# awslabs/aws-c-compression

Measured on AMD Instinct MI355X. Metric: GiB/s input consumed, encode+decode, 1 GiB random bytes; % HBM roofline, higher is better.
Workload: dtype u8

## Files before the change

aws-c-compression_amd/csrc/hip/decode_sync_kernels.hip:

```cpp
#include "decode_common.hpp"
#include "launch_common.hpp"

namespace {


template <u32 NS>
__device__ __forceinline__ void dec_sync_chunk(
    const hufd_tables &tb,
    const hufd_dec_item *items,
    const u32 *chunk_item,
    const u8 *d_in,
    u16 *fn_tab,
    u16 *cp_tab,
    u32 *chunk_fn,
    u8 *chunk_regular,
    u32 c) {

    const u32 ns = tb.n_states;
    u32 *timg = reinterpret_cast<u32 *>(dyn_lds);
    u16 *ftab = reinterpret_cast<u16 *>(timg);
    u32 *gtab = timg + kChunkWords;
    u16 *lut = reinterpret_cast<u16 *>(gtab + kGroups * ns);

    const u32 lane = threadIdx.x;
// ... 108 lines not shown
    __syncthreads();
    HUFD_STAMP(0, 4);
#pragma unroll
    for (u32 s = 0; s < NS; ++s) {
        if (s < ns) {
            ftab[s * HUFD_DEC_LANES + lane] = fn[s];
            fn_tab[((u64)c * ns + s) * HUFD_DEC_LANES + lane] = fn[s];
        }
    }
    {
        u16 *cp = cp_tab + (u64)c * kCpRows * HUFD_DEC_LANES + lane;
#pragma unroll
        for (u32 qq = 0; qq + 1 < kQuarters; ++qq) {
            const u32 tail = ref_steps - cp_steps[qq];
            cp[qq * HUFD_DEC_LANES] =
                (u16)(cp_ok[qq] ? 0x8000u | ((cp_pos[qq] - (qq + 1) * kQuarterBits) << 11) | tail : 0u);
        }
        u32 merged = 0;
#pragma unroll
        for (u32 s = 0; s < NS; ++s) {
            merged |= (have_ref && pos[s] != kDead) ? 1u << s : 0u;
        }
        const u32 common = have_ref ? (ref_stop ? kExitStop : ref_exit) : kExitNoRef;
        cp[(kQuarters - 1) * HUFD_DEC_LANES] = (u16)(merged | (common << 12));
    }
    __syncthreads();

    if (lane < kGroups * ns) {
        const u32 g = lane / ns, start = lane % ns;
        gtab[g * ns + start] = wide_pack(chain_fold(kGroupLanes, start, [&](u32 i, u32 stt) {
            return widen(ftab[stt * HUFD_DEC_LANES + g * kGroupLanes + i]);
        }));
    }
    __syncthreads();
    if (lane < ns) {
        chunk_fn[(u64)c * ns + lane] =
            wide_pack(chain_fold(kGroups, lane, [&](u32 g, u32 stt) { return gtab[g * ns + stt]; }));
    }
    HUFD_STAMP(0, 5);
}

template <u32 NS>
__global__ __launch_bounds__(HUFD_DEC_LANES) void dec_sync_kernel(
    hufd_tables tb,
    const hufd_dec_item *items,
    const u32 *chunk_item,
    u32 n_chunks,
    const u8 *d_in,
    u16 *fn_tab,
    u16 *cp_tab,
    u32 *chunk_fn,
    u8 *chunk_regular,
    const u32 *list,
    const u32 *list_count,
    u32 *clear ) {
    if (clear && blockIdx.x == 0 && threadIdx.x == 0) {
        clear[HUFK_DEC_COUNT_EMIT] = 0;
        clear[HUFK_DEC_COUNT_DENSE] = 0;
    }
    const u32 n = list ? *list_count : n_chunks;
    for (u32 i = blockIdx.x; i < n; i += gridDim.x) {
        const u32 c = list ? list[i] : i;
        if (list && chunk_regular[c] == kRegularFew) {
            continue;
        }
        dec_sync_chunk<NS>(tb, items, chunk_item, d_in, fn_tab, cp_tab, chunk_fn, chunk_regular, c);
        __syncthreads();
    }
}

template <u32 LB>
struct lean_shared {
    u32 wlut[1u << LB];
    u32 exit_state[HUFD_DEC_LANES];
    u32 sub0[kFastMaxMeet + 4];
    u32 wave_sum[HUFD_DEC_LANES / 64];
    u32 bad;
    u32 pad[3];
    u16 hops[1u << LB];
};



constexpr u32 kOneRecs = 9;
__device__ __host__ constexpr u32 one_rec_row(u32 j) {
    return j == 0 ? 6u : j == 1 ? 8u : j == 2 ? 10u : j == 3 ? 12u : j == 4 ? 16u : j == 5 ? 20u : j == 6 ? 24u : j == 7 ? 28u : 32u;
}
constexpr u32 kOneMaxMerge = kSubWords;
constexpr u32 kOneMaxMerge0 = kSubWords;
constexpr u32 kOneRecs0 = kOneRecs;
constexpr u32 kOneGarbageRow = 4, kOneGarbageDead = 48;

__device__ __host__ constexpr u32 one_rec_index(u32 row) {
    u32 at = kOneRecs;
    for (u32 j = 0; j < kOneRecs; ++j) {
        at = one_rec_row(j) == row ? j : at;
    }
    return at;
}

struct one_walk {
    u32 thr, mask;
    static constexpr u32 kPos = 0xFFu;
    __device__ __forceinline__ one_walk(u32 lut_bits) {
        thr = 64 + 31;
        mask = ((1u << lut_bits) - 1u) << 2;
    }
    __device__ __forceinline__ u32 state_at(u32 k) const {
        return thr + 32 - k;
    }
    __device__ __forceinline__ u32 offset_of(u32 state) const {
        return thr + 32 - (state & kPos);
    }
    static __device__ __forceinline__ u32 count_of(u32 state) {
        return state >> 19;
    }
    static __device__ __forceinline__ u32 dead_of(u32 state) {
        return (state >> 8) & 0x7FFu;
    }
    static __device__ __forceinline__ u32 entry_of(u32 len) {
        return len ? (1u << 19) - len : (1u << 8) - 1u;
    }
    template <u32 LB>
    static __device__ __forceinline__ u32 shifted(u32 before, u32 word) {
        return funnel(before, word, 31u - LB);
    }
    __device__ __forceinline__ u32 look(u32 state, u32 xh, u32 xl, u32 table) const {
        return lds_word_at((funnel_by_low5(xh, xl, state) & mask) | table);
    }
    template <u32 SURE>
    __device__ __forceinline__ u32 row(u32 state, u32 xh, u32 xl, u32 table) const {
#pragma unroll
        for (u32 i = 0; i < SURE; ++i) {
            state += look(state, xh, xl, table);
        }
        return byte_rows_uncertain(state, xh, xl, table, mask, thr);
    }
};

template <u32 LB>
struct one_shared {
    u32 wlut[1u << LB];
    u32 exit_state[HUFD_DEC_LANES];
    u32 sub0[kSubWords + 4];
    u32 last0;
    u32 tiny[kTailWords];
    u32 wave_sum[HUFD_DEC_LANES / 64];
    u32 bad;
    u32 decided0;
    u32 moved;
    u32 bad_mine;

};

template <u32 LB, u32 SURE, bool TAIL = false>
__global__ __launch_bounds__(HUFD_DEC_LANES, 8) void dec_sync_one_kernel(
    hufd_tables tb,
    const hufd_chunk_rec *chunk_rec,
    const u32 *tail_chunks,
    const u8 *d_in,
    u16 *fn_tab,
    u16 *cp_tab,
    u32 *chunk_fn,
    u16 *lane_count,
    u8 *chunk_regular,
    u32 *tail_entry,
    u32 *slow_list,
    u32 *slow_count,
    u32 *long_list,
    u32 *long_count) {
    constexpr bool FOLLOW = false;
    const u32 c = TAIL ? wave_uniform(tail_chunks[blockIdx.x]) : blockIdx.x;
#include "decode_sync_one_body.inc"
}

template <u32 LB, u32 SURE>
__global__ __launch_bounds__(HUFD_DEC_LANES, 8) void dec_sync_one_mixed_kernel(
    hufd_tables tb,
    const hufd_chunk_rec *chunk_rec,
    const u32 *tail_chunks,
    u32 n_tail,
    const u8 *d_in,
    u16 *fn_tab,
    u16 *cp_tab,
    u32 *chunk_fn,
    u16 *lane_count,
    u8 *chunk_regular,
    u32 *tail_entry,
    u32 *slow_list,
    u32 *slow_count,
    u32 *long_list,
    u32 *long_count) {
    if (blockIdx.x < n_tail) {
        constexpr bool TAIL = true, FOLLOW = true;
        const u32 c = wave_uniform(tail_chunks[blockIdx.x]);
#include "decode_sync_one_body.inc"
    } else {
        constexpr bool TAIL = false, FOLLOW = false;
        const u32 c = blockIdx.x - n_tail;
#include "decode_sync_one_body.inc"
    }
}




template <u32 LB>
struct pack_shared {
    u32 wlut[1u << LB];
    u32 exit_state[HUFD_DEC_LANES];
    u32 sub0[kPackMaxSlots][kFastMaxMeet + 4];
    u32 sum[kPackMaxSlots];
    u32 bad[kPackMaxSlots];
    u32 alive[kPackMaxSlots];
    u32 meet0[kPackMaxSlots];
    u32 tail0[kPackMaxSlots];
    u16 hops[1u << LB];
};

template <u32 LB, u32 SURE>
__global__ __launch_bounds__(HUFD_DEC_LANES, 6) void dec_sync_pack_kernel(
    hufd_tables tb,
    const hufd_chunk_rec *chunk_rec,
    const u32 *tail_chunks,
    u32 n_tail,
    u32 width,
    const u8 *d_in,
    u16 *fn_tab,
    u16 *cp_tab,
    u32 *chunk_fn,
    u16 *lane_count,
    u8 *chunk_regular,
    u32 *tail_entry,
    u32 *long_list,
    u32 *long_count) {
// ... 998 lines not shown
```

aws-c-compression_amd/csrc/hip/decode_sync_one_body.inc:

```

    static_assert(TAIL || !FOLLOW, "only a chunk its stream ends in has an end to follow");
    HUFD_STAMP(0, 0);
    one_shared<LB> &sh = *reinterpret_cast<one_shared<LB> *>(dyn_lds);
    const u32 ns = tb.n_states;
    const u32 lane = threadIdx.x;
    const hufd_chunk_rec rec = chunk_rec[c];
    const u64 valid = rec.valid;
    const u8 *src = d_in + rec.src_off;
    if (!TAIL && valid < (u64)HUFD_DEC_CHUNK_BYTES + 8u) {
        return;
    }
    const u32 n_full = !TAIL ? HUFD_DEC_LANES : (valid >= 8u ? (u32)((valid - 8u) / HUFD_DEC_SUB_BYTES) : 0u);
    const bool active = !TAIL || lane < n_full;
    if (TAIL && n_full == 0 && tb.lut_bits <= HUFD_DEC_MAX_LUT_BITS) {
        if (lane == 0) {
            chunk_regular[c] = 3;
        }
        if (FOLLOW) {
            u16 *lut = reinterpret_cast<u16 *>(sh.wlut);
            for (u32 i = lane; i < (1u << tb.lut_bits); i += HUFD_DEC_LANES) {
                lut[i] = tb.dec_lut[i];
            }
            __syncthreads();
            if (lane == 0) {
                u32 *tiny = sh.tiny;
                load_be32_run(tiny, src, valid, kTailWords);
                const bool only = rec.entry_bit != HUFD_NONE32;
                for (u32 st = only ? rec.entry_bit : 0u; st < (only ? rec.entry_bit + 1u : ns); ++st) {
                    u32 stop_pos = 0, stop_why = 0;
                    const tail_walk tw = tail_follow(tiny, lut, tb.lut_bits, st, (u32)(valid * 8), 2 * HUFD_DEC_SUB_BITS, nullptr, &stop_pos, &stop_why);
                    chunk_fn[(u64)c * ns + st] = wide_pack(true, 0, tw.count[0] + tw.count[1]);
                }
            }
        }
        return;
    }
    const one_walk ow(LB);
    u32 table = lds_offset_of(sh.wlut);
    opaque(table);
    const bool eligible = n_full >= 1 && tb.lut_bits <= LB && tb.max_bits <= HUFD_DEC_MAX_LUT_BITS &&
                          row_walk(LB, tb.max_bits).sure >= SURE && (table & ((4u << LB) - 1u)) == 0;
    if (!eligible) {
        if (lane == 0) {
            chunk_regular[c] = 0;
            long_list[atomicAdd(long_count, 1u)] = c;
        }
        return;
    }
    u16 *cp = cp_tab + (u64)c * kCpRows * HUFD_DEC_LANES + lane;
    constexpr u32 kLutPerLane = (1u << LB) / HUFD_DEC_LANES, kLutBatch = 4;
    const auto table_share = [&](u32 j0) {
        u32 lut_raw[kLutBatch];
#pragma unroll
        for (u32 j = 0; j < kLutBatch; ++j) {
            lut_raw[j] = tb.dec_lut[(lane + (j0 + j) * HUFD_DEC_LANES) >> (LB - tb.lut_bits)];
        }
#pragma unroll
        for (u32 j = 0; j < kLutBatch; ++j) {
            sh.wlut[lane + (j0 + j) * HUFD_DEC_LANES] = one_walk::entry_of(lut_raw[j] & 0xFFu);
        }
    };
    if (TAIL && lane >= kWave && (lane & ~(kWave - 1)) >= n_full) {
#pragma unroll
        for (u32 j0 = 0; j0 < kLutPerLane; j0 += kLutBatch) {
            table_share(j0);
        }
        if (!FOLLOW || (lane != n_full && lane != n_full + 1)) {
#pragma unroll
            for (u32 qq = 0; qq + 1 < kQuarters; ++qq) {
                cp[qq * HUFD_DEC_LANES] = 0;
            }
            lane_count[(u64)c * HUFD_DEC_LANES + lane] = 0;
            cp[(kQuarters - 1) * HUFD_DEC_LANES] = (u16)(kExitStop << 12);
        }
        return;
    }
    u32 w[kFastRows];
    {
        const u32 mine = active ? lane : 0u;
        const unaligned_uint4 *line = reinterpret_cast<const unaligned_uint4 *>(src + (u64)mine * HUFD_DEC_SUB_BYTES);
#pragma unroll
        for (u32 q = 0; q < kSubWords / 4; ++q) {
            const unaligned_uint4 v = line[q];
            w[4 * q + 0] = v.x;
            w[4 * q + 1] = v.y;
            w[4 * q + 2] = v.z;
            w[4 * q + 3] = v.w;
        }
        w[kSubWords] = reinterpret_cast<const unaligned_u32 *>(src + (u64)(mine + 1) * HUFD_DEC_SUB_BYTES)->x;
    }
#pragma unroll
    for (u32 j0 = 0; j0 < kLutPerLane; j0 += kLutBatch) {
        table_share(j0);
    }
    if (lane == 0) {
        sh.bad = 0;
        sh.decided0 = 0;
        sh.moved = 0;
        sh.bad_mine = 0;
#pragma unroll
        for (u32 wv = 0; wv < HUFD_DEC_LANES / kWave; ++wv) {
            sh.wave_sum[wv] = 0;
        }
    }
    {
        u32 behind = __builtin_bswap32(w[kFastRows - 1]);
#pragma unroll
        for (u32 r = kFastRows - 1; r >= 1; --r) {
            const u32 front = __builtin_bswap32(w[r - 1]);
            w[r] = one_walk::shifted<LB>(front, behind);
            behind = front;
        }
        w[0] = one_walk::shifted<LB>(0u, behind);
    }
    if (lane == 0) {
#pragma unroll
        for (u32 r = 0; r <= kOneMaxMerge0; ++r) {
            sh.sub0[r] = w[r];
        }
    }
    __syncthreads();
    HUFD_STAMP(0, 1);
    HUFD_STAMP(0, 2);

    u32 kept_r[kOneRecs + kQuarters - 1];
#pragma unroll
    for (u32 q = 0; q < kOneRecs + kQuarters - 1; ++q) {
        kept_r[q] = 0;
    }
    auto kept_set = [&](u32 q, u32 v) { kept_r[q] = v; };
    auto kept_get = [&](u32 q) -> u32 { return kept_r[q]; };

    u32 state = ow.state_at(0);
    bool hopeless = false;
#pragma unroll
    for (u32 r = 0; r < kSubWords; ++r) {
        if (!hopeless) {
            if (one_rec_index(r) < kOneRecs) {
                kept_set(one_rec_index(r), state);
            }
            if (r != 0 && r % (kSubWords / kQuarters) == 0) {
                kept_set(kOneRecs + r / (kSubWords / kQuarters) - 1, state);
            }
            state = ow.template row<SURE>(state, w[r], w[r + 1], table) + 32u;
            if (r + 1 == kOneGarbageRow) {
                hopeless = __any(active && one_walk::dead_of(state) > kOneGarbageDead);
            }
        }
    }
    const u32 last = state;
    kept_set(kOneRecs - 1, last);
    if (lane == 0) {
        sh.last0 = last;
    }
    u32 ref_exit = ow.offset_of(last);
    bool ok = !hopeless;
    bool ok_mine = !active || ref_exit < ns;
    sh.exit_state[lane] = ref_exit;
    HUFD_STAMP(0, 3);
    __syncthreads();
    HUFD_STAMP(0, 4);

    u32 entry = lane ? sh.exit_state[lane - 1] : 0u;
    u32 count = 0, meet_row = 0;
    u32 head_cp[kQuarters - 1] = {0, 0, 0};
    {
        u32 st = ow.state_at(entry < ns ? entry : 0u);
        bool met = !active || lane == 0;
        u32 h_at = 0, r_at = 0;
        bool done = false;
        constexpr u32 kInRegisters = 24;
#pragma unroll
        for (u32 r = 0; r <= kInRegisters; ++r) {
            if (!done && !hopeless) {
                if (r != 0 && r % (kSubWords / kQuarters) == 0) {
                    head_cp[r / (kSubWords / kQuarters) - 1] = st;
                }
                if (one_rec_index(r) < kOneRecs) {
                    const u32 there = kept_get(one_rec_index(r));
                    if (!met && ((st ^ there) & one_walk::kPos) == 0) {
                        met = true;
                        h_at = st;
                        r_at = there;
                        meet_row = r;
                    }
                    done = __all(met);
                    if (one_rec_index(r) == 0) {
                        if (!done) {
                            hopeless = __popcll(__ballot(!met)) > kWave - kWave / 8;
                        }
                    }
                }
                if (r < kInRegisters) {
                    if (!done && !hopeless) {
                        st = ow.template row<SURE>(st, w[r], w[r + 1], table) + 32u;
                    }
                }
            }
        }
        if (!done && !hopeless) {
            const u8 *mine = src + (u64)(active ? lane : 0u) * HUFD_DEC_SUB_BYTES;
            u32 word = __builtin_bswap32(reinterpret_cast<const unaligned_u32 *>(mine + 4 * kInRegisters)->x);
            u32 hi = one_walk::shifted<LB>(__builtin_bswap32(reinterpret_cast<const unaligned_u32 *>(mine + 4 * (kInRegisters - 1))->x), word);
            for (u32 r = kInRegisters; r < kSubWords && !done; ++r) {
                const u32 next = __builtin_bswap32(reinterpret_cast<const unaligned_u32 *>(mine + 4 * (r + 1))->x);
                const u32 lo = one_walk::shifted<LB>(word, next);
                word = next;
                st = ow.template row<0>(st, hi, lo, table) + 32u;
                hi = lo;
                if (r + 1 == one_rec_row(kOneRecs - 2) || r + 1 == one_rec_row(kOneRecs - 1)) {
                    const u32 there = r + 1 == one_rec_row(kOneRecs - 2) ? kept_get(kOneRecs - 2) : kept_get(kOneRecs - 1);
                    if (!met && ((st ^ there) & one_walk::kPos) == 0) {
                        met = true;
                        h_at = st;
                        r_at = there;
                        meet_row = r + 1;
                    }
                    done = __all(met);
                }
            }
        }
        if (active && lane && !hopeless && !met && entry < ns) {
            met = true;
            h_at = st;
            r_at = last;
            meet_row = kSubWords;
            ref_exit = ow.offset_of(st);
            sh.exit_state[lane] = ref_exit;
            sh.moved = 1;
        }
        if (active && lane) {
            ok_mine = !hopeless && met && entry < ns && ref_exit < ns && one_walk::dead_of(h_at) == 0 &&
                      one_walk::dead_of(last) == one_walk::dead_of(r_at);
            count = one_walk::count_of(h_at) + one_walk::count_of(last) - one_walk::count_of(r_at);
        }
    }

    HUFD_STAMP(0, 7);
    {
        const u32 wsum0 = wave_sum(lane ? count : 0u);
        if ((lane & (kWave - 1)) == 0) {
            sh.wave_sum[lane / kWave] = wsum0;
        }
        if (!ok) {
            sh.bad = 1;
        }
        if (!ok_mine) {
            sh.bad_mine = 1;
        }
    }
    __syncthreads();
    const bool stay = sh.moved != 0;
    auto lane_records = [&]() {
        if (active) {
#pragma unroll
            for (u32 qq = 0; qq + 1 < kQuarters; ++qq) {
                const u32 boundary = (qq + 1) * (kSubWords / kQuarters);
                bool have = boundary >= meet_row;
                const u32 at_boundary = kept_get(kOneRecs + qq);
                u32 tail = one_walk::count_of(last) - one_walk::count_of(at_boundary), bits = ow.offset_of(at_boundary);
                if (!have && lane != 0) {
                    tail = count - one_walk::count_of(head_cp[qq]);
                    bits = ow.offset_of(head_cp[qq]);
                    have = true;
                }
                cp[qq * HUFD_DEC_LANES] = (u16)(have ? 0x8000u | (bits << 11) | tail : 0u);
            }
        } else if (!FOLLOW || (lane != n_full && lane != n_full + 1)) {
#pragma unroll
            for (u32 qq = 0; qq + 1 < kQuarters; ++qq) {
                cp[qq * HUFD_DEC_LANES] = 0;
            }
            lane_count[(u64)c * HUFD_DEC_LANES + lane] = 0;
            cp[(kQuarters - 1) * HUFD_DEC_LANES] = (u16)(kExitStop << 12);
        }
        if (TAIL && lane + 1 == n_full) {
            tail_entry[c] = ref_exit;
        }
    };
    if (!stay && lane >= kWave) {
        if (!sh.bad && !sh.bad_mine) {
            lane_records();
            if (active) {
                lane_count[(u64)c * HUFD_DEC_LANES + lane] = (u16)count;
                cp[(kQuarters - 1) * HUFD_DEC_LANES] = (u16)((1u << entry) | (ref_exit << 12));
            }
        }
        return;
    }
    u32 cand_count = 0, cand_dead = 0, meet_row0 = 0, ref_count0 = 0;
    bool cand_reached = false;
    u64 cand_alive = 0;
    if (lane < kWave) {
        constexpr u32 kTwin = kWave - 1;
        const bool twin = lane == kTwin;
        const u32 last0 = sh.last0;
        u32 st = ow.state_at(lane < ns ? lane : 0u);
        const u32 only = rec.entry_bit;
        bool dd = only == HUFD_NONE32 ? lane >= ns : lane != only, met = false;
        u32 c_at = 0, r_at = 0;
        u32 at0 = st, latest = 0;
        u32 hi = sh.sub0[0];
        for (u32 r = 0; !hopeless; ++r) {
            const u32 there = __shfl(st, kTwin);
            const bool now = !twin && !dd && !met && ((st ^ there) & one_walk::kPos) == 0 && one_walk::dead_of(last0) == one_walk::dead_of(there);
            if (now) {
                met = true;
                c_at = st;
                r_at = there;
            }
            if (__any(now)) {
                at0 = there;
                latest = r;
            }
            if (__all(dd || met || twin) || r == kSubWords) {
                break;
            }
            const u32 lo = sh.sub0[r + 1];
            if (twin) {
                st = ow.template row<SURE>(st, hi, lo, table);
            } else if (!dd && !met) {
                const u32 before = st;
                st = ow.template row<SURE>(st, hi, lo, table);
                if (one_walk::dead_of(st)) {
                    st = before;
                    for (;;) {
                        const u32 e = ow.look(st, hi, lo, table);
                        if (e == one_walk::entry_of(0)) {
                            break;
                        }
                        st += e;
                    }
                    dd = true;
                    cand_dead = one_walk::count_of(st);
                }
            }
            st += 32u;
            hi = lo;
        }
        const bool decided = !hopeless && __all(dd || met || twin);
        cand_reached = met && lane < ns;
        cand_alive = __ballot(cand_reached);
        meet_row0 = latest;
        cand_count = one_walk::count_of(c_at) + one_walk::count_of(last0) - one_walk::count_of(r_at);
        if (lane == 0) {
            sh.decided0 = decided;
        }
        ok = ok && decided && cand_alive != 0;
        if (lane == 0) {
            meet_row = meet_row0;
            ref_count0 = one_walk::count_of(last0) - one_walk::count_of(at0);
        }
    }

    HUFD_STAMP(0, 5);
    if (!ok) {
        sh.bad = 1;
    }
    if (stay) {
        __syncthreads();
    }
    if (!stay && sh.bad_mine) {
        sh.bad = 1;
    }
    if (stay && !sh.bad) {
        constexpr u32 kRounds = 4;
        u32 round = 0;
        for (; round < kRounds; ++round) {
            __syncthreads();
            if (lane == 0) {
                sh.moved = 0;
            }
            __syncthreads();
            const u32 entry_now = lane ? sh.exit_state[lane - 1] : 0u;
            if (active && lane && entry_now != entry) {
                entry = entry_now;
                bool fine = entry < ns;
                if (fine) {
                    const u8 *mine = src + (u64)lane * HUFD_DEC_SUB_BYTES;
                    u32 st = ow.state_at(entry), h_at = 0, r_at = 0;
                    bool met = false;
                    u32 word = __builtin_bswap32(reinterpret_cast<const unaligned_u32 *>(mine)->x);
                    u32 hi = one_walk::shifted<LB>(0u, word);
                    for (u32 r = 0;; ++r) {
#pragma unroll
                        for (u32 qq = 0; qq + 1 < kQuarters; ++qq) {
                            head_cp[qq] = r == (qq + 1) * (kSubWords / kQuarters) ? st : head_cp[qq];
                        }
                        const u32 j = one_rec_index(r);
                        u32 there = 0;
#pragma unroll
                        for (u32 q = 0; q < kOneRecs; ++q) {
                            there = j == q ? kept_get(q) : there;
                        }
                        if (j < kOneRecs && ((st ^ there) & one_walk::kPos) == 0) {
                            met = true;
                            h_at = st;
                            r_at = there;
                            meet_row = r;
                        }
                        if (met || r == kSubWords) {
                            break;
                        }
                        const u32 next = __builtin_bswap32(reinterpret_cast<const unaligned_u32 *>(mine + 4 * (r + 1))->x);
                        const u32 lo = one_walk::shifted<LB>(word, next);
                        word = next;
                        st = ow.template row<0>(st, hi, lo, table) + 32u;
                        hi = lo;
                    }
                    if (!met) {
                        h_at = st;
                        r_at = last;
                        meet_row = kSubWords;
                    }
                    const u32 exit_now = met ? ow.offset_of(last) : ow.offset_of(st);
                    if (exit_now != ref_exit) {
                        ref_exit = exit_now;
                        sh.exit_state[lane] = exit_now;
                        sh.moved = 1;
                    }
                    fine = ref_exit < ns && one_walk::dead_of(h_at) == 0 && one_walk::dead_of(last) == one_walk::dead_of(r_at);
                    count = one_walk::count_of(h_at) + one_walk::count_of(last) - one_walk::count_of(r_at);
                }
                ok_mine = fine;
            }
            __syncthreads();
            if (!sh.moved) {
                break;
            }
        }
        if (round == kRounds || !ok_mine) {
            sh.bad = 1;
        }
        const u32 wsum_now = wave_sum(lane ? count : 0u);
        if ((lane & (kWave - 1)) == 0) {
            sh.wave_sum[lane / kWave] = wsum_now;
        }
        __syncthreads();
    }
    if (sh.bad) {
        if (lane == 0) {
            chunk_regular[c] = 0;
            if (TAIL || !sh.decided0) {
                long_list[atomicAdd(long_count, 1u)] = c;
            } else {
                slow_list[atomicAdd(slow_count, 1u)] = c;
            }
        }
        return;
    }

    u16 *fn_out = fn_tab + (u64)c * ns * HUFD_DEC_LANES;
    lane_records();
    if (active) {
        const u32 total = lane ? count : ref_count0;
        lane_count[(u64)c * HUFD_DEC_LANES + lane] = (u16)total;
        cp[(kQuarters - 1) * HUFD_DEC_LANES] = (u16)((lane ? 1u << entry : (u32)cand_alive) | (ref_exit << 12));
    }
    if (lane == 0) {
        chunk_regular[c] = TAIL ? 2 : 1;
    }
    u32 follow_exit = 0, follow_count = 0, follow_stop = 2;
    if (FOLLOW && lane < kWave) {
        u16 *lut = reinterpret_cast<u16 *>(sh.wlut);
        u32 *words = sh.wlut + (1u << LB) / 2;
        const u32 entry_t = sh.exit_state[n_full - 1];
        wave_step();
        for (u32 i = lane; i < (1u << tb.lut_bits); i += kWave) {
            lut[i] = tb.dec_lut[i];
        }
        tail_walk tw = {{0, 0}, 0, 2};
        if (lane == 0) {
            const u8 *tsrc = src + (u64)n_full * HUFD_DEC_SUB_BYTES;
            const u64 tail_bytes = valid - (u64)n_full * HUFD_DEC_SUB_BYTES;
            load_be32_run(words, tsrc, tail_bytes, kTailWords);
        }
        wave_step();
        if (lane == 0) {
            const u64 tail_bytes = valid - (u64)n_full * HUFD_DEC_SUB_BYTES;
            const u32 limit = (n_full + 1 < HUFD_DEC_LANES ? 2u : 1u) * HUFD_DEC_SUB_BITS;
            u32 stop_pos = 0, stop_why = 0;
            tw = tail_follow(words, lut, tb.lut_bits, entry_t, (u32)(tail_bytes * 8), limit, nullptr, &stop_pos, &stop_why);
            for (u32 k = 0; k < 2; ++k) {
                const u32 ln = n_full + k;
                if (ln >= HUFD_DEC_LANES) {
                    break;
                }
                u16 *cpl = cp_tab + (u64)c * kCpRows * HUFD_DEC_LANES + ln;
                const bool reached = k == 0 || tw.stop != 0;
#pragma unroll
                for (u32 qq = 0; qq + 1 < kQuarters; ++qq) {
                    cpl[qq * HUFD_DEC_LANES] = 0;
                }
                if (reached) {
                    const u32 my_entry = k == 0 ? entry_t : tw.exit;
                    const bool stops_here = tw.stop == k;
                    lane_count[(u64)c * HUFD_DEC_LANES + ln] = (u16)tw.count[k];
                    fn_out[(u64)my_entry * HUFD_DEC_LANES + ln] =
                        stops_here ? fn_pack(true, 0, tw.count[k] & 0x7FFu) : fn_pack(false, tw.exit, tw.count[k] & 0x7FFu);
                    cpl[(kQuarters - 1) * HUFD_DEC_LANES] = (u16)((1u << my_entry) | ((stops_here ? kExitStop : tw.exit) << 12));
                } else {
                    lane_count[(u64)c * HUFD_DEC_LANES + ln] = 0;
                    cpl[(kQuarters - 1) * HUFD_DEC_LANES] = (u16)(kExitStop << 12);
                }
            }
        }
        follow_exit = __shfl(tw.exit, 0);
        follow_count = __shfl(tw.count[0] + tw.count[1], 0);
        follow_stop = __shfl(tw.stop, 0);
    }
    if (lane < ns) {
        u32 rest = 0;
#pragma unroll
        for (u32 wv = 0; wv < HUFD_DEC_LANES / kWave; ++wv) {
            rest += sh.wave_sum[wv];
        }
        const u32 first_exit = sh.exit_state[0];
        const u32 last_exit = sh.exit_state[HUFD_DEC_LANES - 1];
        fn_out[(u64)lane * HUFD_DEC_LANES] =
            cand_reached ? fn_pack(false, first_exit, cand_count & 0x7FFu) : fn_pack(true, 0, cand_dead);
        const bool stops = follow_stop != 2u;
        chunk_fn[(u64)c * ns + lane] =
            cand_reached ? (FOLLOW ? wide_pack(stops, stops ? 0u : follow_exit, cand_count + rest + follow_count)
                                   : wide_pack(false, TAIL ? 0u : last_exit, cand_count + rest))
                         : wide_pack(true, 0, cand_dead);
    }
    HUFD_STAMP(0, 6);
```

aws-c-compression_amd/csrc/hip/kernels_common.hpp:

```cpp
#ifndef HUFFMAN_AMD_KERNELS_COMMON_HPP
#define HUFFMAN_AMD_KERNELS_COMMON_HPP
#include <hip/hip_runtime.h>
#include <numeric>
#include <type_traits>

#include <pthread.h>
#include <stdint.h>
#include <stdio.h>
#include <stdlib.h>

#include "device_types.h"
#include "huffman_kernels.h"

namespace {


typedef unsigned int u32;
typedef uint64_t u64;
typedef unsigned short u16;
typedef unsigned char u8;

constexpr u32 kWave = 64;

__device__ __forceinline__ u32 wave_uniform(u32 x) {
#if defined(__HIP_DEVICE_COMPILE__)
    return __builtin_amdgcn_readfirstlane(x);
#else
    return x;
#endif
}
constexpr u64 kNoBit = ~0ull;

HIP_DYNAMIC_SHARED(__attribute__((aligned(16))) unsigned char, dyn_lds)

#ifdef HUFD_STAMPS
__device__ unsigned long long *hufd_stamp_rows;
#define HUFD_STAMP_MAX_WG 131072u
#define HUFD_STAMP(kernel, phase)                                                                                      \
    do {                                                                                                               \
        if (threadIdx.x == 0 && blockIdx.x < HUFD_STAMP_MAX_WG) {                                                      \
            hufd_stamp_rows[((u64)(kernel)*HUFD_STAMP_MAX_WG + blockIdx.x) * 8 + (phase)] =                            \
                (unsigned long long)clock64();                                                                         \
        }                                                                                                              \
    } while (0)
#define HUFD_STAMP_DECL __shared__ unsigned long long hufd_stamp_acc[8];
#define HUFD_STAMP_ZERO                                                                                                \
    do {                                                                                                               \
        if (threadIdx.x < 8) {                                                                                         \
            hufd_stamp_acc[threadIdx.x] = 0;                                                                           \
        }                                                                                                              \
    } while (0)
#ifdef HUFD_STAMPS_WHY
#define HUFD_STAMP_TIMED(phase) ((phase) < 3 || (phase) > 5)
#else
#define HUFD_STAMP_TIMED(phase) true
#endif
#define HUFD_STAMP_ADD(kernel, phase)                                                                                  \
    do {                                                                                                               \
        if (threadIdx.x == 0 && HUFD_STAMP_TIMED(phase)) {                                                             \
            hufd_stamp_acc[phase] += (unsigned long long)clock64();                                                    \
        }                                                                                                              \
    } while (0)
#define HUFD_STAMP_COUNT(phase, n)                                                                                     \
    do {                                                                                                               \
        if (threadIdx.x == 0) {                                                                                        \
            hufd_stamp_acc[phase] += (unsigned long long)(n);                                                          \
        }                                                                                                              \
    } while (0)
#define HUFD_STAMP_FLUSH(kernel)                                                                                       \
    do {                                                                                                               \
        if (threadIdx.x < 8 && blockIdx.x < HUFD_STAMP_MAX_WG) {                                                       \
            hufd_stamp_rows[((u64)(kernel)*HUFD_STAMP_MAX_WG + blockIdx.x) * 8 + threadIdx.x] =                        \
                hufd_stamp_acc[threadIdx.x];                                                                           \
        }                                                                                                              \
    } while (0)
#else
#define HUFD_STAMP(kernel, phase)
#define HUFD_STAMP_ADD(kernel, phase)
#define HUFD_STAMP_DECL
#define HUFD_STAMP_ZERO
#define HUFD_STAMP_COUNT(phase, n)
#define HUFD_STAMP_FLUSH(kernel)
#endif

struct __attribute__((packed, aligned(1))) unaligned_uint4 {
    u32 x, y, z, w;
};
struct __attribute__((packed, aligned(1))) unaligned_u32 {
    u32 x;
};

__device__ __forceinline__ u32 round16(u32 x) {
    return (x + 15u) & ~15u;
}



__device__ __forceinline__ void opaque(u32 &x) {
#if defined(__HIP_DEVICE_COMPILE__)
    asm volatile("" : "+v"(x));
#else
    (void)x;
#endif
}

__device__ __forceinline__ hufd_enc_seg uniform_seg(const hufd_enc_seg *p) {
    hufd_enc_seg d = *p;
#if defined(__HIP_DEVICE_COMPILE__)
    const u32 lo = __builtin_amdgcn_readfirstlane((u32)d.in_off);
    const u32 hi = __builtin_amdgcn_readfirstlane((u32)(d.in_off >> 32));
    d.in_off = ((u64)hi << 32) | lo;
    d.len = __builtin_amdgcn_readfirstlane(d.len);
    d.item = __builtin_amdgcn_readfirstlane(d.item);
    d.index = __builtin_amdgcn_readfirstlane(d.index);
    d.flags = __builtin_amdgcn_readfirstlane(d.flags);
    d.next_len = __builtin_amdgcn_readfirstlane(d.next_len);
#endif
    return d;
}

__device__ __forceinline__ void barrier_lds() {
#if defined(__HIP_DEVICE_COMPILE__)
    asm volatile("s_waitcnt lgkmcnt(0)" ::: "memory");
    __builtin_amdgcn_s_barrier();
    asm volatile("" ::: "memory");
#else
    __syncthreads();
#endif
}

__device__ __forceinline__ void lds_dma16(const void *global_src, void *lds_dst) {
#if defined(__HIP_DEVICE_COMPILE__)
    __builtin_amdgcn_global_load_lds(
        (const __attribute__((address_space(1))) void *)global_src, (__attribute__((address_space(3))) void *)lds_dst,
        16, 0, 0);
#else
    memcpy(lds_dst, global_src, 16);
#endif
}

__device__ __forceinline__ u32 funnel(u32 hi, u32 lo, u32 shift ) {
#if defined(__HIP_DEVICE_COMPILE__)
    return __builtin_amdgcn_alignbit(hi, lo, shift);
#else
    return (u32)(((((u64)hi) << 32) | lo) >> shift);
#endif
}

__device__ __forceinline__ u32 funnel_by_low5(u32 hi, u32 lo, u32 word) {
#if defined(__HIP_DEVICE_COMPILE__)
    return __builtin_amdgcn_alignbit(hi, lo, word);
#else
    return (u32)(((((u64)hi) << 32) | lo) >> (word & 31u));
#endif
}

__device__ __forceinline__ u32 word_load_now(const u32 *p) {
#if defined(__HIP_DEVICE_COMPILE__)
    u32 v;
    asm volatile("global_load_dword %0, %1, off sc1\n\ts_waitcnt vmcnt(0)" : "=&v"(v) : "v"(p) : "memory");
    return v;
#else
    return *p;
#endif
}
// ... 212 lines not shown
```

Before: 659.0.

## Hand late-converging lanes to a finisher wave and redo only changed successors

Each lane now walks its sub-block only up to an early row, and lanes that have not yet synchronised with the reference path park their state, remaining words and kept checkpoints in a shared slot table. One finisher wave then completes those walks in a compact batch, so the other waves can exit early instead of idling on divergent long walks. The re-walk after an exit-state change is replaced by a redo worklist that only touches successor lanes, and per-lane counts are gathered through a shared array instead of per-wave sums. The cost is extra LDS use, overflow fallbacks to the slow path when too many lanes are handed over or redone, and added serialisation on one wave.

Result: no change. 653.2 (-0.9%).

```diff
diff --git a/aws-c-compression_amd/csrc/hip/decode_sync_kernels.hip b/aws-c-compression_amd/csrc/hip/decode_sync_kernels.hip
--- a/aws-c-compression_amd/csrc/hip/decode_sync_kernels.hip
+++ b/aws-c-compression_amd/csrc/hip/decode_sync_kernels.hip
@@ -214,9 +214,19 @@
 
 
 
-constexpr u32 kOneRecs = 9;
+#ifndef HUFD_ONE_HAND_ROW
+#define HUFD_ONE_HAND_ROW 4u
+#endif
+constexpr u32 kOneHandRow = HUFD_ONE_HAND_ROW;
+static_assert(kOneHandRow >= 3 && kOneHandRow <= 5, "boundaries 2 and S, or 2, 4 and 5");
+constexpr u32 kOneStageRecs = kOneHandRow == 5 ? 3 : 2;
+constexpr u32 kOneRecs = kOneStageRecs + 9;
 __device__ __host__ constexpr u32 one_rec_row(u32 j) {
-    return j == 0 ? 6u : j == 1 ? 8u : j == 2 ? 10u : j == 3 ? 12u : j == 4 ? 16u : j == 5 ? 20u : j == 6 ? 24u : j == 7 ? 28u : 32u;
+    if (j < kOneStageRecs) {
+        return j + 1 == kOneStageRecs ? kOneHandRow : 2u * (j + 1u);
+    }
+    const u32 k = j - kOneStageRecs;
+    return k == 0 ? 6u : k == 1 ? 8u : k == 2 ? 10u : k == 3 ? 12u : k == 4 ? 16u : k == 5 ? 20u : k == 6 ? 24u : k == 7 ? 28u : 32u;
 }
 constexpr u32 kOneMaxMerge = kSubWords;
 constexpr u32 kOneMaxMerge0 = kSubWords;
@@ -269,6 +279,16 @@
         return byte_rows_uncertain(state, xh, xl, table, mask, thr);
     }
 };
+
+constexpr u32 kOneHandLast = 16;
+constexpr u32 kOneHandWords = kOneHandLast - kOneHandRow + 1;
+constexpr u32 kOneHandKept = kOneRecs - kOneStageRecs;
+constexpr u32 kOneSlotWords = 2 + kOneHandWords + kOneHandKept;
+__device__ __host__ constexpr u32 one_slots(u32 lut_bits) {
+    return lut_bits > 10 ? HUFD_DEC_LANES / 4 : HUFD_DEC_LANES / 2;
+}
+constexpr u32 kOneRedoMax = 64;
+constexpr u32 kOneLaneBad = 0xFFFFu;
 
 template <u32 LB>
 struct one_shared {
@@ -277,12 +297,14 @@
     u32 sub0[kSubWords + 4];
     u32 last0;
     u32 tiny[kTailWords];
-    u32 wave_sum[HUFD_DEC_LANES / 64];
     u32 bad;
     u32 decided0;
     u32 moved;
-    u32 bad_mine;
-
+    u32 n_handed;
+    u32 n_redo[2];
+    u16 redo[2][kOneRedoMax];
+    u16 info[HUFD_DEC_LANES];
+    u32 hand[kOneSlotWords][one_slots(LB)];
 };
 
 template <u32 LB, u32 SURE, bool TAIL = false>
diff --git a/aws-c-compression_amd/csrc/hip/decode_sync_one_body.inc b/aws-c-compression_amd/csrc/hip/decode_sync_one_body.inc
--- a/aws-c-compression_amd/csrc/hip/decode_sync_one_body.inc
+++ b/aws-c-compression_amd/csrc/hip/decode_sync_one_body.inc
@@ -36,6 +36,7 @@
         return;
     }
     const one_walk ow(LB);
+    constexpr u32 kOneSlots = one_slots(LB);
     u32 table = lds_offset_of(sh.wlut);
     opaque(table);
     const bool eligible = n_full >= 1 && tb.lut_bits <= LB && tb.max_bits <= HUFD_DEC_MAX_LUT_BITS &&
@@ -73,6 +74,7 @@
             lane_count[(u64)c * HUFD_DEC_LANES + lane] = 0;
             cp[(kQuarters - 1) * HUFD_DEC_LANES] = (u16)(kExitStop << 12);
         }
+        sh.info[lane] = 0;
         return;
     }
     u32 w[kFastRows];
@@ -97,11 +99,9 @@
         sh.bad = 0;
         sh.decided0 = 0;
         sh.moved = 0;
-        sh.bad_mine = 0;
-#pragma unroll
-        for (u32 wv = 0; wv < HUFD_DEC_LANES / kWave; ++wv) {
-            sh.wave_sum[wv] = 0;
-        }
+        sh.n_handed = 0;
+        sh.n_redo[0] = 0;
+        sh.n_redo[1] = 0;
     }
     {
         u32 behind = __builtin_bswap32(w[kFastRows - 1]);
@@ -161,21 +161,16 @@
     __syncthreads();
     HUFD_STAMP(0, 4);
 
-    u32 entry = lane ? sh.exit_state[lane - 1] : 0u;
+    const u32 entry = lane ? sh.exit_state[lane - 1] : 0u;
     u32 count = 0, meet_row = 0;
-    u32 head_cp[kQuarters - 1] = {0, 0, 0};
+    bool late = false;
     {
         u32 st = ow.state_at(entry < ns ? entry : 0u);
-        bool met = !active || lane == 0;
+        bool met = !active || lane == 0 || entry >= ns;
         u32 h_at = 0, r_at = 0;
-        bool done = false;
-        constexpr u32 kInRegisters = 24;
-#pragma unroll
-        for (u32 r = 0; r <= kInRegisters; ++r) {
-            if (!done && !hopeless) {
-                if (r != 0 && r % (kSubWords / kQuarters) == 0) {
-                    head_cp[r / (kSubWords / kQuarters) - 1] = st;
-                }
+#pragma unroll
+        for (u32 r = 0; r <= kOneHandRow; ++r) {
+            if (!hopeless) {
                 if (one_rec_index(r) < kOneRecs) {
                     const u32 there = kept_get(one_rec_index(r));
                     if (!met && ((st ^ there) & one_walk::kPos) == 0) {
@@ -184,52 +179,30 @@
                         r_at = there;
                         meet_row = r;
                     }
-                    done = __all(met);
-                    if (one_rec_index(r) == 0) {
-                        if (!done) {
-                            hopeless = __popcll(__ballot(!met)) > kWave - kWave / 8;
-                        }
-                    }
-                }
-                if (r < kInRegisters) {
-                    if (!done && !hopeless) {
-                        st = ow.template row<SURE>(st, w[r], w[r + 1], table) + 32u;
-                    }
-                }
-            }
-        }
-        if (!done && !hopeless) {
-            const u8 *mine = src + (u64)(active ? lane : 0u) * HUFD_DEC_SUB_BYTES;
-            u32 word = __builtin_bswap32(reinterpret_cast<const unaligned_u32 *>(mine + 4 * kInRegisters)->x);
-            u32 hi = one_walk::shifted<LB>(__builtin_bswap32(reinterpret_cast<const unaligned_u32 *>(mine + 4 * (kInRegisters - 1))->x), word);
-            for (u32 r = kInRegisters; r < kSubWords && !done; ++r) {
-                const u32 next = __builtin_bswap32(reinterpret_cast<const unaligned_u32 *>(mine + 4 * (r + 1))->x);
-                const u32 lo = one_walk::shifted<LB>(word, next);
-                word = next;
-                st = ow.template row<0>(st, hi, lo, table) + 32u;
-                hi = lo;
-                if (r + 1 == one_rec_row(kOneRecs - 2) || r + 1 == one_rec_row(kOneRecs - 1)) {
-                    const u32 there = r + 1 == one_rec_row(kOneRecs - 2) ? kept_get(kOneRecs - 2) : kept_get(kOneRecs - 1);
-                    if (!met && ((st ^ there) & one_walk::kPos) == 0) {
-                        met = true;
-                        h_at = st;
-                        r_at = there;
-                        meet_row = r + 1;
-                    }
-                    done = __all(met);
-                }
-            }
-        }
-        if (active && lane && !hopeless && !met && entry < ns) {
-            met = true;
-            h_at = st;
-            r_at = last;
-            meet_row = kSubWords;
-            ref_exit = ow.offset_of(st);
-            sh.exit_state[lane] = ref_exit;
-            sh.moved = 1;
-        }
-        if (active && lane) {
+                }
+                if (r < kOneHandRow) {
+                    st = ow.template row<SURE>(st, w[r], w[r + 1], table) + 32u;
+                }
+            }
+        }
+        late = !met && !hopeless;
+        if (late) {
+            const u32 slot = atomicAdd(&sh.n_handed, 1u);
+            if (slot < kOneSlots) {
+                u32 *f = &sh.hand[0][slot];
+                f[0] = lane | (entry << 16);
+                f[kOneSlots] = st;
+#pragma unroll
+                for (u32 j = 0; j < kOneHandWords; ++j) {
+                    f[(2 + j) * kOneSlots] = w[kOneHandRow + j];
+                }
+#pragma unroll
+                for (u32 q = 0; q < kOneHandKept; ++q) {
+                    f[(2 + kOneHandWords + q) * kOneSlots] = kept_get(kOneStageRecs + q);
+                }
+            }
+            ok_mine = true;
+        } else if (active && lane) {
             ok_mine = !hopeless && met && entry < ns && ref_exit < ns && one_walk::dead_of(h_at) == 0 &&
                       one_walk::dead_of(last) == one_walk::dead_of(r_at);
             count = one_walk::count_of(h_at) + one_walk::count_of(last) - one_walk::count_of(r_at);
@@ -237,36 +210,47 @@
     }
 
     HUFD_STAMP(0, 7);
-    {
-        const u32 wsum0 = wave_sum(lane ? count : 0u);
-        if ((lane & (kWave - 1)) == 0) {
-            sh.wave_sum[lane / kWave] = wsum0;
-        }
-        if (!ok) {
-            sh.bad = 1;
-        }
-        if (!ok_mine) {
-            sh.bad_mine = 1;
-        }
+    sh.info[lane] = (u16)(ok_mine ? count : kOneLaneBad);
+    if (!ok) {
+        sh.bad = 1;
     }
     __syncthreads();
-    const bool stay = sh.moved != 0;
-    auto lane_records = [&]() {
-        if (active) {
-#pragma unroll
-            for (u32 qq = 0; qq + 1 < kQuarters; ++qq) {
-                const u32 boundary = (qq + 1) * (kSubWords / kQuarters);
-                bool have = boundary >= meet_row;
-                const u32 at_boundary = kept_get(kOneRecs + qq);
-                u32 tail = one_walk::count_of(last) - one_walk::count_of(at_boundary), bits = ow.offset_of(at_boundary);
-                if (!have && lane != 0) {
-                    tail = count - one_walk::count_of(head_cp[qq]);
-                    bits = ow.offset_of(head_cp[qq]);
-                    have = true;
-                }
-                cp[qq * HUFD_DEC_LANES] = (u16)(have ? 0x8000u | (bits << 11) | tail : 0u);
-            }
-        } else if (!FOLLOW || (lane != n_full && lane != n_full + 1)) {
+    const u32 n_handed = wave_uniform(sh.n_handed);
+    if (n_handed > kOneSlots) {
+        if (lane == 0) {
+            chunk_regular[c] = 0;
+            long_list[atomicAdd(long_count, 1u)] = c;
+            HUFD_HANDOVER_NOTE(c, n_handed, 0);
+        }
+        return;
+    }
+    auto quarters_out = [&](u16 *cpl, bool first_lane, u32 met_at, u32 total, u32 last_, const u32(&at_q)[kQuarters - 1],
+                            const u32(&head)[kQuarters - 1]) {
+#pragma unroll
+        for (u32 qq = 0; qq + 1 < kQuarters; ++qq) {
+            const u32 boundary = (qq + 1) * (kSubWords / kQuarters);
+            bool have = boundary >= met_at;
+            u32 tail = one_walk::count_of(last_) - one_walk::count_of(at_q[qq]), bits = ow.offset_of(at_q[qq]);
+            if (!have && !first_lane) {
+                tail = total - one_walk::count_of(head[qq]);
+                bits = ow.offset_of(head[qq]);
+                have = true;
+            }
+            cpl[qq * HUFD_DEC_LANES] = (u16)(have ? 0x8000u | (bits << 11) | tail : 0u);
+        }
+    };
+    const u32 my_q[kQuarters - 1] = {kept_get(kOneRecs), kept_get(kOneRecs + 1), kept_get(kOneRecs + 2)};
+    const u32 no_head[kQuarters - 1] = {0, 0, 0};
+    static_assert(kOneHandRow < kSubWords / kQuarters, "a lane that met in stage 1 has passed no checkpoint");
+    if (!sh.bad) {
+        if (active && lane && !late) {
+            quarters_out(cp, false, meet_row, count, last, my_q, no_head);
+            lane_count[(u64)c * HUFD_DEC_LANES + lane] = (u16)count;
+            cp[(kQuarters - 1) * HUFD_DEC_LANES] = (u16)((1u << entry) | (ref_exit << 12));
+            if (TAIL && lane + 1 == n_full) {
+                tail_entry[c] = ref_exit;
+            }
+        } else if (!active && (!FOLLOW || (lane != n_full && lane != n_full + 1))) {
 #pragma unroll
             for (u32 qq = 0; qq + 1 < kQuarters; ++qq) {
                 cp[qq * HUFD_DEC_LANES] = 0;
@@ -274,20 +258,125 @@
             lane_count[(u64)c * HUFD_DEC_LANES + lane] = 0;
             cp[(kQuarters - 1) * HUFD_DEC_LANES] = (u16)(kExitStop << 12);
         }
-        if (TAIL && lane + 1 == n_full) {
-            tail_entry[c] = ref_exit;
-        }
-    };
-    if (!stay && lane >= kWave) {
-        if (!sh.bad && !sh.bad_mine) {
-            lane_records();
-            if (active) {
-                lane_count[(u64)c * HUFD_DEC_LANES + lane] = (u16)count;
-                cp[(kQuarters - 1) * HUFD_DEC_LANES] = (u16)((1u << entry) | (ref_exit << 12));
-            }
-        }
-        return;
-    }
+    }
+    const u32 fin_wave = TAIL ? (n_full - 1) / kWave : HUFD_DEC_LANES / kWave - 1;
+    const bool finisher = lane / kWave == fin_wave;
+    if (lane >= kWave && !finisher) {
+        return;
+    }
+    const u32 n_lanes = TAIL ? n_full : HUFD_DEC_LANES;
+
+    if (finisher) {
+        constexpr u32 kQ0 = one_rec_index(kSubWords / kQuarters) - kOneStageRecs, kQ1 = one_rec_index(2 * kSubWords / kQuarters) - kOneStageRecs,
+                      kQ2 = one_rec_index(3 * kSubWords / kQuarters) - kOneStageRecs;
+        static_assert(kQ0 < kOneHandKept && kQ1 < kOneHandKept && kQ2 < kOneHandKept, "the quarter boundaries are kept ones");
+        for (u32 base = 0; base < n_handed; base += kWave) {
+            const u32 k = base + (lane & (kWave - 1));
+            const bool have = k < n_handed;
+            const u32 *f = &sh.hand[0][have ? k : 0u];
+            const u32 who = f[0];
+            const u32 ln = who & 0xFFFFu, ent = who >> 16;
+            u32 st = f[kOneSlots];
+            u32 hw[kOneHandWords], hk[kOneHandKept];
+#pragma unroll
+            for (u32 j = 0; j < kOneHandWords; ++j) {
+                hw[j] = f[(2 + j) * kOneSlots];
+            }
+#pragma unroll
+            for (u32 q = 0; q < kOneHandKept; ++q) {
+                hk[q] = f[(2 + kOneHandWords + q) * kOneSlots];
+            }
+            const u32 last_l = hk[kOneHandKept - 1];
+            bool met = !have, done = false;
+            u32 h_at = 0, r_at = 0, met_at = 0;
+            u32 head[kQuarters - 1] = {0, 0, 0};
+#pragma unroll
+            for (u32 r = kOneHandRow; r <= kOneHandLast; ++r) {
+                if (!done) {
+                    if (r % (kSubWords / kQuarters) == 0) {
+                        head[r / (kSubWords / kQuarters) - 1] = st;
+                    }
+                    if (r > kOneHandRow && one_rec_index(r) < kOneRecs) {
+                        const u32 there = hk[one_rec_index(r) - kOneStageRecs];
+                        if (!met && ((st ^ there) & one_walk::kPos) == 0) {
+                            met = true;
+                            h_at = st;
+                            r_at = there;
+                            met_at = r;
+                        }
+                        done = __all(met);
+                    }
+                    if (r < kOneHandLast) {
+                        if (!done) {
+                            st = ow.template row<SURE>(st, hw[r - kOneHandRow], hw[r - kOneHandRow + 1], table) + 32u;
+                        }
+                    }
+                }
+            }
+            if (!done) {
+                const u8 *mine = src + (u64)ln * HUFD_DEC_SUB_BYTES;
+                u32 word = __builtin_bswap32(reinterpret_cast<const unaligned_u32 *>(mine + 4 * kOneHandLast)->x);
+                u32 hi = one_walk::shifted<LB>(__builtin_bswap32(reinterpret_cast<const unaligned_u32 *>(mine + 4 * (kOneHandLast - 1))->x), word);
+                for (u32 r = kOneHandLast; r < kSubWords && !done; ++r) {
+                    const u32 next = __builtin_bswap32(reinterpret_cast<const unaligned_u32 *>(mine + 4 * (r + 1))->x);
+                    const u32 lo = one_walk::shifted<LB>(word, next);
+                    word = next;
+                    st = ow.template row<0>(st, hi, lo, table) + 32u;
+                    hi = lo;
+#pragma unroll
+                    for (u32 qq = 0; qq + 1 < kQuarters; ++qq) {
+                        head[qq] = r + 1 == (qq + 1) * (kSubWords / kQuarters) ? st : head[qq];
+                    }
+                    const u32 j = one_rec_index(r + 1);
+                    if (j < kOneRecs) {
+                        u32 there = 0;
+#pragma unroll
+                        for (u32 q = 0; q < kOneHandKept; ++q) {
+                            there = j == kOneStageRecs + q ? hk[q] : there;
+                        }
+                        if (!met && ((st ^ there) & one_walk::kPos) == 0) {
+                            met = true;
+                            h_at = st;
+                            r_at = there;
+                            met_at = r + 1;
+                        }
+                        done = __all(met);
+                    }
+                }
+            }
+            u32 exit_l = ow.offset_of(last_l);
+            if (have && !met) {
+                h_at = st;
+                r_at = last_l;
+                met_at = kSubWords;
+                exit_l = ow.offset_of(st);
+                sh.exit_state[ln] = exit_l;
+                sh.moved = 1;
+                if (ln + 1 < n_lanes) {
+                    const u32 at = atomicAdd(&sh.n_redo[0], 1u);
+                    if (at < kOneRedoMax) {
+                        sh.redo[0][at] = (u16)(ln + 1);
+                    } else {
+                        sh.bad = 1;
+                    }
+                }
+            }
+            if (have) {
+                const bool fine = exit_l < ns && one_walk::dead_of(h_at) == 0 && one_walk::dead_of(last_l) == one_walk::dead_of(r_at);
+                const u32 total = one_walk::count_of(h_at) + one_walk::count_of(last_l) - one_walk::count_of(r_at);
+                u16 *cpl = cp_tab + (u64)c * kCpRows * HUFD_DEC_LANES + ln;
+                const u32 at_q[kQuarters - 1] = {hk[kQ0], hk[kQ1], hk[kQ2]};
+                quarters_out(cpl, false, met_at, total, last_l, at_q, head);
+                lane_count[(u64)c * HUFD_DEC_LANES + ln] = (u16)total;
+                cpl[(kQuarters - 1) * HUFD_DEC_LANES] = (u16)((1u << ent) | (exit_l << 12));
+                if (TAIL && ln + 1 == n_full) {
+                    tail_entry[c] = exit_l;
+                }
+                sh.info[ln] = (u16)(fine ? total : kOneLaneBad);
+            }
+        }
+    }
+
     u32 cand_count = 0, cand_dead = 0, meet_row0 = 0, ref_count0 = 0;
     bool cand_reached = false;
     u64 cand_alive = 0;
@@ -357,50 +446,39 @@
     if (!ok) {
         sh.bad = 1;
     }
-    if (stay) {
-        __syncthreads();
-    }
-    if (!stay && sh.bad_mine) {
-        sh.bad = 1;
-    }
-    if (stay && !sh.bad) {
+    __syncthreads();
+    if (sh.moved && !sh.bad) {
         constexpr u32 kRounds = 4;
         u32 round = 0;
         for (; round < kRounds; ++round) {
+            const u32 now = round & 1u;
+            const u32 n_redo = wave_uniform(sh.n_redo[now]);
+            if (n_redo == 0) {
+                break;
+            }
+            if (lane == 0) {
+                sh.n_redo[now ^ 1u] = 0;
+            }
+            u32 who = 0, entry_now = 0;
+            const bool walks = finisher && (lane & (kWave - 1)) < n_redo;
+            if (walks) {
+                who = sh.redo[now][lane & (kWave - 1)];
+                entry_now = sh.exit_state[who - 1];
+            }
             __syncthreads();
-            if (lane == 0) {
-                sh.moved = 0;
-            }
-            __syncthreads();
-            const u32 entry_now = lane ? sh.exit_state[lane - 1] : 0u;
-            if (active && lane && entry_now != entry) {
-                entry = entry_now;
-                bool fine = entry < ns;
+            if (walks) {
+                bool fine = entry_now < ns;
+                u32 total = 0;
                 if (fine) {
-                    const u8 *mine = src + (u64)lane * HUFD_DEC_SUB_BYTES;
-                    u32 st = ow.state_at(entry), h_at = 0, r_at = 0;
-                    bool met = false;
+                    const u8 *mine = src + (u64)who * HUFD_DEC_SUB_BYTES;
+                    u32 st = ow.state_at(entry_now);
+                    u32 head[kQuarters - 1] = {0, 0, 0};
                     u32 word = __builtin_bswap32(reinterpret_cast<const unaligned_u32 *>(mine)->x);
                     u32 hi = one_walk::shifted<LB>(0u, word);
-                    for (u32 r = 0;; ++r) {
+                    for (u32 r = 0; r < kSubWords; ++r) {
 #pragma unroll
                         for (u32 qq = 0; qq + 1 < kQuarters; ++qq) {
-                            head_cp[qq] = r == (qq + 1) * (kSubWords / kQuarters) ? st : head_cp[qq];
-                        }
-                        const u32 j = one_rec_index(r);
-                        u32 there = 0;
-#pragma unroll
-                        for (u32 q = 0; q < kOneRecs; ++q) {
-                            there = j == q ? kept_get(q) : there;
-                        }
-                        if (j < kOneRecs && ((st ^ there) & one_walk::kPos) == 0) {
-                            met = true;
-                            h_at = st;
-                            r_at = there;
-                            meet_row = r;
-                        }
-                        if (met || r == kSubWords) {
-                            break;
+                            head[qq] = r == (qq + 1) * (kSubWords / kQuarters) ? st : head[qq];
                         }
                         const u32 next = __builtin_bswap32(reinterpret_cast<const unaligned_u32 *>(mine + 4 * (r + 1))->x);
                         const u32 lo = one_walk::shifted<LB>(word, next);
@@ -408,37 +486,57 @@
                         st = ow.template row<0>(st, hi, lo, table) + 32u;
                         hi = lo;
                     }
-                    if (!met) {
-                        h_at = st;
-                        r_at = last;
-                        meet_row = kSubWords;
-                    }
-                    const u32 exit_now = met ? ow.offset_of(last) : ow.offset_of(st);
-                    if (exit_now != ref_exit) {
-                        ref_exit = exit_now;
-                        sh.exit_state[lane] = exit_now;
-                        sh.moved = 1;
-                    }
-                    fine = ref_exit < ns && one_walk::dead_of(h_at) == 0 && one_walk::dead_of(last) == one_walk::dead_of(r_at);
-                    count = one_walk::count_of(h_at) + one_walk::count_of(last) - one_walk::count_of(r_at);
-                }
-                ok_mine = fine;
+                    const u32 exit_now = ow.offset_of(st);
+                    if (exit_now != sh.exit_state[who]) {
+                        sh.exit_state[who] = exit_now;
+                        if (who + 1 < n_lanes) {
+                            const u32 at = atomicAdd(&sh.n_redo[now ^ 1u], 1u);
+                            if (at < kOneRedoMax) {
+                                sh.redo[now ^ 1u][at] = (u16)(who + 1);
+                            } else {
+                                sh.bad = 1;
+                            }
+                        }
+                    }
+                    fine = exit_now < ns && one_walk::dead_of(st) == 0;
+                    total = one_walk::count_of(st);
+                    u16 *cpl = cp_tab + (u64)c * kCpRows * HUFD_DEC_LANES + who;
+                    quarters_out(cpl, false, kSubWords, total, st, head, head);
+                    lane_count[(u64)c * HUFD_DEC_LANES + who] = (u16)total;
+                    cpl[(kQuarters - 1) * HUFD_DEC_LANES] = (u16)((1u << entry_now) | (exit_now << 12));
+                    if (TAIL && who + 1 == n_full) {
+                        tail_entry[c] = exit_now;
+                    }
+                }
+                sh.info[who] = (u16)(fine ? total : kOneLaneBad);
             }
             __syncthreads();
-            if (!sh.moved) {
-                break;
-            }
-        }
-        if (round == kRounds || !ok_mine) {
+        }
+        if (round == kRounds && sh.n_redo[round & 1u] != 0) {
             sh.bad = 1;
         }
-        const u32 wsum_now = wave_sum(lane ? count : 0u);
-        if ((lane & (kWave - 1)) == 0) {
-            sh.wave_sum[lane / kWave] = wsum_now;
-        }
         __syncthreads();
     }
-    if (sh.bad) {
+    if (lane >= kWave) {
+        return;
+    }
+    u32 rest;
+    {
+        const u16 *mine = &sh.info[lane * (HUFD_DEC_LANES / kWave)];
+        u32 sum = 0;
+        bool wrong = false;
+#pragma unroll
+        for (u32 j = 0; j < HUFD_DEC_LANES / kWave; ++j) {
+            const u32 v = mine[j];
+            wrong = wrong || v == kOneLaneBad;
+            sum += v;
+        }
+        rest = wave_sum(sum);
+        if (__any(wrong)) {
+            ok = false;
+        }
+    }
+    if (!ok || sh.bad) {
         if (lane == 0) {
             chunk_regular[c] = 0;
             if (TAIL || !sh.decided0) {
@@ -446,19 +544,21 @@
             } else {
                 slow_list[atomicAdd(slow_count, 1u)] = c;
             }
+            HUFD_HANDOVER_NOTE(c, n_handed, 0);
         }
         return;
     }
 
     u16 *fn_out = fn_tab + (u64)c * ns * HUFD_DEC_LANES;
-    lane_records();
-    if (active) {
-        const u32 total = lane ? count : ref_count0;
-        lane_count[(u64)c * HUFD_DEC_LANES + lane] = (u16)total;
-        cp[(kQuarters - 1) * HUFD_DEC_LANES] = (u16)((lane ? 1u << entry : (u32)cand_alive) | (ref_exit << 12));
-    }
     if (lane == 0) {
+        quarters_out(cp, true, meet_row, 0u, last, my_q, no_head);
+        lane_count[(u64)c * HUFD_DEC_LANES] = (u16)ref_count0;
+        cp[(kQuarters - 1) * HUFD_DEC_LANES] = (u16)((u32)cand_alive | (ref_exit << 12));
+        if (TAIL && n_full == 1) {
+            tail_entry[c] = ref_exit;
+        }
         chunk_regular[c] = TAIL ? 2 : 1;
+        HUFD_HANDOVER_NOTE(c, n_handed, TAIL ? 2 : 1);
     }
     u32 follow_exit = 0, follow_count = 0, follow_stop = 2;
     if (FOLLOW && lane < kWave) {
@@ -510,11 +610,6 @@
         follow_stop = __shfl(tw.stop, 0);
     }
     if (lane < ns) {
-        u32 rest = 0;
-#pragma unroll
-        for (u32 wv = 0; wv < HUFD_DEC_LANES / kWave; ++wv) {
-            rest += sh.wave_sum[wv];
-        }
         const u32 first_exit = sh.exit_state[0];
         const u32 last_exit = sh.exit_state[HUFD_DEC_LANES - 1];
         fn_out[(u64)lane * HUFD_DEC_LANES] =
diff --git a/aws-c-compression_amd/csrc/hip/kernels_common.hpp b/aws-c-compression_amd/csrc/hip/kernels_common.hpp
--- a/aws-c-compression_amd/csrc/hip/kernels_common.hpp
+++ b/aws-c-compression_amd/csrc/hip/kernels_common.hpp
@@ -11,6 +11,31 @@
 
 #include "device_types.h"
 #include "huffman_kernels.h"
+
+#if !defined(__HIP__) && !defined(__HIPCC__)
+#include <vector>
+struct hufd_emu_note {
+    unsigned chunk, handed, regular;
+};
+inline std::vector<hufd_emu_note> &hufd_emu_note_list() {
+    static std::vector<hufd_emu_note> notes;
+    return notes;
+}
+extern "C" __attribute__((used, visibility("default"))) inline size_t hufd_emu_handover_notes(unsigned *out, size_t cap) {
+    std::vector<hufd_emu_note> &notes = hufd_emu_note_list();
+    size_t n = 0;
+    for (; n < notes.size() && n < cap; ++n) {
+        out[3 * n + 0] = notes[n].chunk;
+        out[3 * n + 1] = notes[n].handed;
+        out[3 * n + 2] = notes[n].regular;
+    }
+    const size_t all = notes.size();
+    notes.clear();
+    return all;
+}
+#define HUFD_HANDOVER_NOTE(chunk, handed, regular)                                                                     \
+    hufd_emu_note_list().push_back(hufd_emu_note{(unsigned)(chunk), (unsigned)(handed), (unsigned)(regular)})
+#endif
 
 namespace {
 
@@ -81,6 +106,18 @@
 #define HUFD_STAMP_ZERO
 #define HUFD_STAMP_COUNT(phase, n)
 #define HUFD_STAMP_FLUSH(kernel)
+#endif
+
+#if defined(HUFD_STAMPS)
+#define HUFD_HANDOVER_NOTE(chunk, handed, regular)                                                                     \
+    do {                                                                                                               \
+        if ((chunk) < HUFD_STAMP_MAX_WG) {                                                                             \
+            hufd_stamp_rows[((u64)HUFD_STAMP_MAX_WG + (chunk)) * 8 + 7] =                                              \
+                ((unsigned long long)(regular) << 32) | (unsigned long long)(handed);                                 \
+        }                                                                                                              \
+    } while (0)
+#elif !defined(HUFD_HANDOVER_NOTE)
+#define HUFD_HANDOVER_NOTE(chunk, handed, regular)
 #endif
 
 struct __attribute__((packed, aligned(1))) unaligned_uint4 {
```
